# andrewhou1/BlindShadowRemoval

Measured on AMD Instinct MI355X. Metric: images/sec at 256x256 batch inference (GSC generator forward), higher is better.
Workload: dtype f32; 1 GPU; BASELINE configs[1]: batch=32 synthetic 256x256x3 per GPU, full GSC generator fp32 (seeded random-init weights in the ckpt-94 variable layout); global_batch=32, height=256, width=256, parallelism=dp1, forwards_in_flight=1, collective=none

## Files before the change

blindshadowremoval_amd/_lib.py:

```python
from __future__ import annotations

import ctypes
import os
from typing import Optional

from . import build as _build
from .build import LIB_PATH

ABI_VERSION = 8
NUM_CLASSES = 7
CLASS_NAMES = ("conv3x3", "convT3x3", "conv1x1", "attention", "conv7", "glue", "convT3x3_ni2")

_lib: Optional[ctypes.CDLL] = None

c_i, c_v, c_sz, c_s = ctypes.c_int, ctypes.c_void_p, ctypes.c_size_t, ctypes.c_char_p
_BS = [c_i, c_i]
_BLOBS = [c_v, c_sz, c_v, c_sz]

SIGNATURES = {
    "bsr_abi_version": (c_i, None),
    "bsr_last_error": (c_s, None),
    "bsr_source_sha": (c_s, None),
    "bsr_create": (c_i, [ctypes.POINTER(c_v), c_i, c_v, c_sz, c_i]),
    "bsr_destroy": (None, [c_v]),
    "bsr_forward": (c_i, [c_v, c_v, c_v, c_i, c_i, c_i, c_v, c_v, c_v, c_v, c_v]),
    "bsr_forward_packed": (c_i, [c_v, c_v, c_v, c_i, c_i, c_i, c_v, c_v, c_v, c_v]),
    "bsr_forward_tsm": (c_i, [c_v, c_v, c_v, c_v, c_i, c_i, c_i, c_i, c_i, c_v, c_v, c_v, c_v, c_v]),
    "bsr_forward_rgb": (c_i, [c_v, c_v, c_v, c_i, c_i, c_i, c_v, c_v]),
    "bsr_workspace_bytes": (c_sz, [c_i, c_i, c_i]),
    "bsr_handle_workspace_bytes": (c_sz, [c_v, c_i, c_i, c_i]),
    "bsr_reserve": (c_i, [c_v, c_i, c_i, c_i]),
    "bsr_probe": (c_i, [c_v, c_s, c_v, c_sz, ctypes.POINTER(c_i * 4), c_v]),
    "bsr_set_timing": (c_i, [c_v, c_i]),
    "bsr_get_timing": (c_i, [c_v, ctypes.POINTER(ctypes.c_float * NUM_CLASSES), ctypes.POINTER(c_i * NUM_CLASSES)]),
    "bsr_timing_launches": (c_i, [c_v]),
    "bsr_timing_entry": (c_i, [c_v, c_i, c_s, c_sz, ctypes.POINTER(ctypes.c_float), ctypes.POINTER(c_i)]),
    "bsr_clock_trace": (c_i, [c_i, c_v, c_i, c_i, c_v, c_v, c_v]),
    "bsr_check_range": (c_i, [c_v, c_v]),
    "bsr_peek_range": (c_i, [c_v]),
    "bsr_debug_attention": (c_i, [c_v, c_v, c_i, c_i, c_v]),
    "bsr_debug_attention_rgb": (c_i, [c_v, c_v, c_i, c_i, c_v]),
    "bsr_debug_attention_dtype": (c_i, [c_v, c_v, c_i, c_i, c_i, c_v]),
    "bsr_debug_attention_qw": (c_i, [c_v, c_v, c_i, c_i, c_i, c_v]),
    "bsr_debug_attention_split": (c_i, [c_v, c_v, c_i, c_i, c_i, c_v]),
    "bsr_debug_attention_kv1": (c_i, [c_v, c_v, c_i, c_i, c_i, c_v]),
    "bsr_debug_split_qkv": (c_i, [c_v, c_v, c_i, c_i, c_v]),
    "bsr_debug_wino_conv": (c_i, [c_v, c_v, c_v, c_v, c_i, c_i, c_i, c_i, c_v]),
    "bsr_debug_wino_filter": (c_i, [c_v, c_v]),
    "bsr_debug_keys_compose": (c_i, [c_v, c_v, c_v, c_v]),
    "bsr_debug_values_compose": (c_i, [c_v, c_v, c_v, c_v, c_v, c_v]),
    "bsr_prep_rows": (c_i, [c_i, c_v, c_sz, c_sz, c_sz, c_i, c_i, c_v, c_v, c_v]),
    "bsr_prep_groups": (c_i, [c_i, c_v, c_sz, c_sz, c_sz, c_i, c_i, c_i, c_v, c_v, c_v]),
    "bsr_png_unfilter": (c_i, [c_i, c_v, c_sz, c_sz, c_i, c_v]),
    "bsr_png_unfilter_tall": (c_i, [c_i, c_v, c_sz, c_sz, c_i, c_v]),
    "bsr_png_file_bytes": (c_sz, [c_i, c_i]),
    "bsr_png_scratch_bytes": (c_sz, [c_i]),
    "bsr_png_encode": (c_i, [c_i, c_v, c_i, c_i, c_i, c_v, c_sz, c_v, c_v]),
    "bsr_png_encode_figs": (c_i, [c_i, c_i, c_v, c_v, c_v, c_v, c_v, c_v, c_i, c_i, c_i, c_v, c_sz, c_v, c_v]),
    "bsr_crop_faces": (c_i, [c_i, c_v, c_sz, c_sz, c_i, c_i, c_v]),
    "bsr_paste_faces": (c_i, [c_i, c_v, c_sz, c_sz, c_i, c_i, c_v, c_i, c_v, c_i, c_v, c_i, c_i, c_v]),
    "bsr_ucb_post_scratch_bytes": (c_sz, _BS),
    "bsr_ucb_post": (c_i, [c_i, c_v, c_v, c_v, c_i, c_i, c_v, c_v, c_v, c_v, c_v, c_v]),
    "bsr_ucb_post_rgb_scratch_bytes": (c_sz, _BS),
    "bsr_ucb_post_rgb": (c_i, [c_i, c_v, c_v, c_v, c_i, c_i, c_v, c_v, c_v, c_v, c_v, c_v]),
    "bsr_ucb_post_tsm_scratch_bytes": (c_sz, _BS),
    "bsr_ucb_post_tsm": (c_i, [c_i, c_v, c_v, c_v, c_i, c_i, c_v, c_v, c_v, c_v, c_v, c_v, c_v]),
    "bsr_sfw_score_scratch_bytes": (c_sz, _BS),
    "bsr_sfw_score": (c_i, [c_i, c_v, c_i, c_i, c_v, c_v, c_v, c_v, c_v, c_v, c_v]),
    "bsr_shadow_synth_scratch_bytes": (c_sz, _BS),
    "bsr_shadow_synth": (c_i, [c_i, c_v, c_v, c_v, c_v, c_v, c_sz, c_i, c_i, c_v, c_v, c_v, c_v, c_v, c_v, c_v]),
    "bsr_train_losses_scratch_bytes": (c_sz, _BS),
    "bsr_train_losses": (c_i, [c_i, c_v, c_v, c_v, c_v, c_v, c_i, c_i, c_v, c_v, c_v, c_v, c_v, c_v, c_v]),
    "bsr_train_losses_grad_scratch_bytes": (c_sz, _BS),
    "bsr_train_losses_grad_offset": (c_sz, [c_i, c_i, c_i]),
    "bsr_train_losses_grad": (c_i, [c_i, c_v, c_v, c_v, c_v, c_v, c_v, c_i, c_i, c_v, c_v, c_v, c_v, c_v, c_v, c_v, c_v]),
    "bsr_disc_blob_bytes": (c_sz, []),
    "bsr_disc_losses_scratch_bytes": (c_sz, _BS),
    "bsr_disc_act_offset": (c_sz, [c_i, c_i, c_i, c_i]),
    "bsr_disc_losses": (c_i, [c_i, c_v, c_sz, c_v, c_v, c_v, c_i, c_i, c_v, c_v, c_v, c_v, c_v]),
    "bsr_disc_dgrad_blob_bytes": (c_sz, []),
    "bsr_disc_grad_scratch_bytes": (c_sz, _BS),
    "bsr_disc_grad_offset": (c_sz, [c_i, c_i, c_i, c_i]),
    "bsr_disc_gen_grad": (c_i, [c_i] + _BLOBS + [c_v, c_v, c_v, c_v, c_i, c_i, c_v, c_v, c_v, c_v, c_v, c_v]),
    "bsr_debug_disc_gen_grad": (c_i, [c_i] + _BLOBS + [c_v, c_v, c_v, c_v, c_i, c_i, c_v, c_v, c_v, c_v, c_v, c_i, c_v]),
    "bsr_disc_wgrad_blob_bytes": (c_sz, []),
    "bsr_disc_wgrad_scratch_bytes": (c_sz, _BS),
    "bsr_disc_wgrad_floats": (c_sz, []),
    "bsr_disc_wgrad_var_offset": (c_sz, [c_i]),
    "bsr_disc_wgrad_offset": (c_sz, [c_i, c_i, c_i, c_i]),
    "bsr_disc_wgrad": (c_i, [c_i] + _BLOBS + [c_v, c_sz, c_v, c_v, c_v, c_i, c_i, c_v, c_v, c_v, c_v, c_v, c_v]),
    "bsr_debug_disc_wgrad": (c_i, [c_i] + _BLOBS + [c_v, c_sz, c_v, c_v, c_v, c_i, c_i, c_v, c_v, c_v, c_v, c_v, c_i, c_v]),
    "bsr_clr_tail_grad_blob_bytes": (c_sz, []),
    "bsr_clr_tail_grad_scratch_bytes": (c_sz, [c_i, c_i, c_i]),
    "bsr_clr_tail_grad_floats": (c_sz, []),
    "bsr_clr_tail_grad_var_offset": (c_sz, [c_i]),
    "bsr_clr_tail_grad_offset": (c_sz, [c_i, c_i, c_i, c_i]),
    "bsr_clr_tail_grad_partials": (c_i, [c_i, c_i, c_i]),
    "bsr_clr_tail_grad": (c_i, [c_i, c_v, c_sz, c_v, c_v, c_i, c_v, c_v, c_i, c_i, c_i, c_v, c_v, c_v, c_i, c_v, c_v]),
    "bsr_debug_clr_tail_grad": (c_i, [c_i, c_v, c_sz, c_v, c_v, c_i, c_v, c_v, c_i, c_i, c_i, c_v, c_v, c_v, c_i, c_v, c_i, c_v]),
    "bsr_last_f": (c_i, [c_v, ctypes.POINTER(c_v), ctypes.POINTER(c_i), ctypes.POINTER(c_i * 4)]),
# ... 76 lines not shown
```

blindshadowremoval_amd/csrc/bsr_api.hip:

```cpp
#include "../../include/bsr_hip.h"

#include <hip/hip_runtime.h>
#include <stdint.h>
#include <stdio.h>
#include <stdlib.h>
#include <string.h>

#include <initializer_list>
#include <string>
#include <type_traits>
#include <unordered_map>
#include <vector>

#include "attention.h"
#include "attention256.h"
#include "attention_h16.h"
#include "conv3_f16.h"
#include "conv_n16.h"
#include "gemm_nloop.h"
#include "glue_kernels.h"
#include "igemm_conv.h"
#include "igemm_h16.h"
#include "png_kernels.h"
#include "prep_kernels.h"
// ... 124 lines not shown
  p.xa = take(cells * v.cs_a, true);
  p.t1 = take(cells * v.d);
  p.t2 = take(cells * v.d);
  for (int i = 0; i < v.nblk; ++i) p.y3[i] = take(cells * v.cs_y3x);
  p.qkv = take(cells * 3 * v.d);
  for (int i = 0; i < v.nblk; ++i) p.att[i] = take(cells * v.d);
  for (int i = 0; i < v.nblk; ++i) p.r[i] = take(cells * (i < 3 ? v.cs_r : v.cs_h), !v.rgb);
  p.xh = take(cells * v.cs_h, true);
  p.ybuf = take(px * v.cs_y);
  p.qh = take(px * v.cs_qh);
  p.f1 = take(px2 / 16 * 128);
  p.f2 = take(px2 / 4 * 96);
  p.cf = take(px2 * CS_CF);
  p.probe = take(px2 / 64 * 2);
  p.reg32 = take(v.tsm ? cells * 4 : 0);
  p.share = take(v.tsm ? cells * 2 * v.c_r : 0);
  p.yh = take(px1 * 3);
  p.con = take(px1 * 3);
  p.total = off;
  return p;
}

}

struct bsr_handle {
  int device = 0;
  float* d_blob = nullptr;
  float* d_wino = nullptr;
  float* d_keys = nullptr;
  float* d_values = nullptr;
  float* att_scratch = nullptr;
  size_t att_scratch_floats = 0;
  std::unordered_map<std::string, LayerW> layers;
  Variant var = kGSC;
  int dtype = BSR_DTYPE_F32;
  float head_bias[2] = {0.f, 0.f};
  const float* tail_w = nullptr;
  const float* clr_gs_w = nullptr;
  float* ws = nullptr;
  size_t ws_floats = 0;
  Plan plan{};
  const float* rgb_tail_w = nullptr;
  const float* rgb_head_b = nullptr;
  int B = 0, H = 0, W = 0;
  bool ran = false;
  bool att_in_lds = false;
  unsigned* range_flag = nullptr;
  bool fuse_heads = true;
  bool conv1_gemm = true;
  bool att_pv1 = false;
  bool conv3_f16 = true;
  bool fuse_attw = true;
  bool wino_conv2 = true;
  bool keys_conv2 = true;
  bool values_conv2 = true;
  bool att_is_o = false;
  bool timing = false;
  std::vector<hipEvent_t> ev;
  std::vector<int> ev_class;
  std::vector<std::string> ev_name;
  size_t ev_used = 0;
};

namespace {

const char* const kRangeMsg =
    "an activation exceeded the fp16 range (|x| >= 65520) in a forward of this 16-bit-mode handle: its outputs are not trustworthy "
    "(inf / NaN where the fp32 path stays finite).  Re-run those inputs on a BSR_DTYPE_F32 handle; bsr_check_range() clears the condition";

constexpr size_t kWinoFloats = 8 * 16 * 128 * 16;
void wino_filter_transform(const float* direct, float* out) {
  static const double G[4][3] = {{1.0, 0.0, 0.0}, {0.5, 0.5, 0.5}, {0.5, -0.5, 0.5}, {0.0, 0.0, 1.0}};
  for (int k = 0; k < 128; ++k)
    for (int n = 0; n < 128; ++n) {
      double t[4][3];
      for (int x = 0; x < 4; ++x)
        for (int b = 0; b < 3; ++b) {
          double acc = 0.0;
          for (int a = 0; a < 3; ++a) acc += G[x][a] * (double)direct[((size_t)((k / 32) * 9 + a * 3 + b) * 128 + n) * 36 + k % 32];
          t[x][b] = acc;
        }
      for (int x = 0; x < 4; ++x)
        for (int y = 0; y < 4; ++y) {
          double acc = 0.0;
          for (int b = 0; b < 3; ++b) acc += t[x][b] * G[y][b];
          out[((size_t)((k / 16) * 16 + 4 * x + y) * 128 + n) * 16 + k % 16] = (float)acc;
        }
    }
}

constexpr int kKeysN = 288 + 256, kKeysNPad = kKeysN + 64, kC3qNPad = 768;
constexpr size_t kKeysFloats = (size_t)4 * kKeysNPad * 36 + kKeysNPad;
void keys_compose(const float* c3q_w, const float* c3q_b, float* out_w, float* out_b) {
  auto src = [&](int k, int n) -> const float& { return c3q_w[((size_t)(k / 32) * kC3qNPad + n) * 36 + k % 32]; };
  memset(out_w, 0, (size_t)4 * kKeysNPad * 36 * sizeof(float));
  memset(out_b, 0, kKeysNPad * sizeof(float));
  for (int ch = 0; ch < 4; ++ch) {
    memcpy(out_w + (size_t)ch * kKeysNPad * 36, c3q_w + (size_t)ch * kC3qNPad * 36, (size_t)288 * 36 * sizeof(float));
    memcpy(out_w + ((size_t)ch * kKeysNPad + 416) * 36, c3q_w + ((size_t)ch * kC3qNPad + 544) * 36, (size_t)128 * 36 * sizeof(float));
  }
  memcpy(out_b, c3q_b, 288 * sizeof(float));
  memcpy(out_b + 416, c3q_b + 544, 128 * sizeof(float));
  for (int m = 0; m < 128; ++m) {
    for (int k = 0; k < 128; ++k) {
      double acc = 0.0;
      for (int c = 0; c < 128; ++c) acc += (double)src(k, 288 + c) * (double)src(m, 416 + c);
// ... 196 lines not shown
      const int most = (tiles + NI - 1) / NI;
      kNSplit = want < 2 ? 2 : (want > most ? most : want);
#ifdef BSR_NL_NSPLIT
      kNSplit = BSR_NL_NSPLIT > most ? most : BSR_NL_NSPLIT;
#endif
    }
    if (image == nullptr) rc = find_layer(h, name, NCH, 1, 36, (tiles + NI - 1) * 32, &l);
    else if (image->nchunk == NCH && image->ldp == 36 && image->n_pad >= (tiles + NI - 1) * 32) l = *image;
    else rc = fail(BSR_ERR_ARG, std::string("layer '") + name + "': the handle's image does not fit the kernel");
    if (rc != BSR_OK) return;
    if (pixels % C::BM != 0) { rc = fail(BSR_ERR_ARG, std::string("layer '") + name + "': pixel count is not a multiple of 128"); return; }
    bsr::ConvArgs a = gemm_args(l, in, in_cs, out, out_cs, n_store, act);
    a.res1 = res1; a.res1_cs = res1_cs; a.res1_c = res1_c;
    a.out2 = out2; a.out2_cs = out2_cs; a.n_split = n_split; a.n_store1 = n_store1; a.out2_gap_at = out2_gap_at; a.out2_gap = out2_gap;
    a.out2_split = (h->dtype != BSR_DTYPE_F32 && out2 != nullptr) ? 1 : 0;
    begin(cls, name);
    if (h->dtype == BSR_DTYPE_F32)
      check(bsr::launch_gemm_nloop<NI, NCH, 0, MINW>(a, pixels, kNSplit, s), name);
    else if constexpr (MINW == 2)
      check(bsr::launch_gemm_nloop<NI, NCH, 2>(a, pixels, kNSplit, s), name);
    else
      rc = fail(BSR_ERR_ARG, std::string("layer '") + name + "': the RGB bottleneck GEMMs are fp32 only");
    end();
  }
  template <int NCH>
  void gemm_all_n(const char* name, const float* in, size_t pixels, float* out) {
    if (rc != BSR_OK) return;
    LayerW l;
    rc = find_layer(h, name, NCH, 1, 36, 128, &l);
    if (rc != BSR_OK) return;
    begin(K_CONV1, name);
    check(bsr::launch_gemm_nloop<4, NCH, 2, 1>(gemm_args(l, in, NCH * 32, out, 128, 128, 1), pixels, 1, s), name);
    end();
  }

  void stem(const float* in, int H, int W, float* out) {
    if (rc != BSR_OK) return;
    LayerW l;
    rc = find_layer(h, "conv1", 1, 7, h->dtype != BSR_DTYPE_F32 ? 36 : 28, 32, &l);
    if (rc != BSR_OK) return;
    bsr::StemArgs a{in, out, l.w, l.b, H, W, 0, 0, 0, h->range_flag};
    begin(K_CONV7, "conv1");
    with_dtype(h->dtype, [&](auto prec, auto half) { check(bsr::launch_stem7<4, prec.value, half.value>(a, h->B, s), "conv1"); });
    end();
  }

  void wino(const char* name, int i, const float* in, int H, int W, float* out, int out_cs = 128) {
    if (rc != BSR_OK) return;
    LayerW l;
    rc = find_layer(h, name, 4, 9, 36, 128, &l);
    if (rc != BSR_OK) return;
    if (H % 4 != 0 || W % 32 != 0) { rc = fail(BSR_ERR_ARG, std::string("layer '") + name + "': feature map is not a multiple of the 4x32 tile"); return; }
    begin(K_CONV3, name);
    check(bsr::launch_wino_conv2(wino_args(in, out, h->d_wino + (size_t)i * kWinoFloats, l.b, H, W, out_cs), h->B, s), name);
    end();
  }

  void conv71(const char* name, const float* in, int in_cs, int k_pad, int H, int W, float* out, int out_cs) {
    if (rc != BSR_OK) return;
    LayerW l;
    rc = find_layer(h, name, k_pad / 32, 7, 36, 32, &l);
    if (rc != BSR_OK) return;
    if (H % 4 != 0 || W % 32 != 0) { rc = fail(BSR_ERR_ARG, std::string("layer '") + name + "': image is not a multiple of the 4x32 tile"); return; }
    bsr::ConvArgs a{};
    a.in = in; a.in_cs = in_cs; a.in_coff = 0; a.H = H; a.W = W;
    a.out = out; a.out_cs = out_cs; a.out_coff = 0; a.Ho = H; a.Wo = W;
    a.w = l.w; a.bias = l.b; a.nchunk = l.nchunk; a.n_pad = l.n_pad; a.n_store = 32;
    a.pad_t = 3; a.pad_l = 0; a.act = 0;
    begin(K_CONV7, name);
    check(bsr::launch_igemm_conv<7, 1, 1, false, 4, 32, 4, 1, 1, 1, 32, 1>(a, h->B, s), name);
    end();
  }

  void heads(const float* y, int H, int W, float* qh, const float* inputs, float* gs, float* mask22, size_t npix) {
    if (rc != BSR_OK) return;
    LayerW l;
    rc = find_layer(h, "heads", 2, 7, 36, 16, &l);
    if (rc != BSR_OK) return;
    if (l.n_pad != 16) { rc = fail(BSR_ERR_BLOB, "layer 'heads' must be packed with n_pad 16"); return; }
    if (H % 8 != 0 || W % 32 != 0) { rc = fail(BSR_ERR_ARG, "layer 'heads': image is not a multiple of its tile"); return; }
    bsr::ConvN16Args a{};
    a.in = y; a.in_cs = 64; a.H = H; a.W = W; a.w = l.w; a.bias = l.b; a.out = qh; a.out_cs = 16; a.act = 0;
    a.pad_t = 3; a.pad_l = 0;
    a.inputs = inputs; a.gs_out = gs; a.mask22 = mask22; a.b_mask = h->head_bias[0]; a.b_con = h->head_bias[1];
    a.range_flag = h->range_flag;
    int resident = 0;
    check(bsr::launch_conv_n16<7, 1, false, false, 2, 0, false, true>(a, h->B, s, &resident), "heads");
    const bool fuse = rc == BSR_OK && h->fuse_heads && bsr::conv_n16_fuse_pays(h->B, H, 8, resident);
    begin(K_CONV7, "heads");
    with_dtype(h->dtype, [&](auto prec, auto half) {
      if (fuse) check(bsr::launch_conv_n16<7, 1, false, false, 2, prec.value, half.value, true>(a, h->B, s), "heads");
      else check(bsr::launch_conv_n16<7, 1, false, false, 2, prec.value, half.value>(a, h->B, s), "heads");
    });
    end();
    if (fuse) return;
    begin(K_GLUE, "heads_post");
    hipLaunchKernelGGL(bsr::heads_post_kernel, dim3((unsigned)((npix + 255) / 256)), dim3(256), 0, s, qh, inputs, h->head_bias[0], h->head_bias[1], gs,
                       mask22, W, npix);
    check(hipGetLastError(), "heads_post");
    end();
  }

  template <int KH, int KW, bool GS, bool TAIL, int RW>
  void conv16(int cls, const char* name, const float* in, int in_cs, int H, int W, float* out, int out_cs, int act, const float* gs,
              const float* inputs, float* con_rgb, float* dif, float* packed = nullptr) {
    if (rc != BSR_OK) return;
    LayerW l;
// ... 43 lines not shown
}

template <typename T>
int read_records(const unsigned char* blob, size_t off, int n, hipStream_t s, std::vector<T>* out) {
  out->resize((size_t)n);
  HIP_TRY(hipMemcpyAsync(out->data(), blob + off, (size_t)n * sizeof(T), hipMemcpyDeviceToHost, s));
  HIP_TRY(hipStreamSynchronize(s));
  return BSR_OK;
}

}

extern "C" {

int bsr_abi_version(void) { return 8; }

#ifndef BSR_SRC_SHA
#define BSR_SRC_SHA "unhashed"
#endif
static const char kSrcShaTag[] = "BSR_SRC_SHA=" BSR_SRC_SHA;
const char* bsr_source_sha(void) { return kSrcShaTag + 12; }

const char* bsr_last_error(void) { return g_last_error.c_str(); }

size_t bsr_workspace_bytes(int B, int H, int W) {
  if (B <= 0 || H <= 0 || W <= 0) return 0;
  return make_plan(B, H, W, kGSC).total * sizeof(float);
}

int bsr_create(bsr_handle** out, int device, const void* packed_weights, size_t nbytes, int dtype) {
  if (out == nullptr || packed_weights == nullptr) return fail(BSR_ERR_ARG, "bsr_create: null argument");
  *out = nullptr;
  if (dtype != BSR_DTYPE_F32 && dtype != BSR_DTYPE_F16 && dtype != BSR_DTYPE_F32X3)
    return fail(BSR_ERR_ARG, "bsr_create: dtype must be BSR_DTYPE_F32, BSR_DTYPE_F16 or BSR_DTYPE_F32X3");
  if (nbytes < sizeof(BlobHeader)) return fail(BSR_ERR_BLOB, "bsr_create: blob shorter than its header");
  const uint8_t* blob = static_cast<const uint8_t*>(packed_weights);
  BlobHeader hd;
  memcpy(&hd, blob, sizeof hd);
  if (hd.magic != kBlobMagic || hd.version != kBlobVersion) return fail(BSR_ERR_BLOB, "bsr_create: bad blob magic/version");
  if ((int)hd.reserved != dtype) return fail(BSR_ERR_BLOB, "bsr_create: the blob was packed for another dtype (pack_generator(weights, dtype) must match bsr_create's dtype)");
  const size_t table_end = sizeof(BlobHeader) + (size_t)hd.n_entries * sizeof(BlobEntry);
  if (table_end > nbytes) return fail(BSR_ERR_BLOB, "bsr_create: blob entry table exceeds blob size");
  DeviceGuard guard(device);
  HIP_TRY(guard.err);
  bsr_handle* h = new bsr_handle();
  h->device = device;
  h->dtype = dtype;
  h->att_pv1 = dtype == BSR_DTYPE_F16;
  const struct { const char* env; bool* on; } switches[] = {{"BSR_FUSE_HEADS", &h->fuse_heads}, {"BSR_FUSE_ATTW", &h->fuse_attw}, {"BSR_CONV3_F16", &h->conv3_f16},
                                                            {"BSR_CONV1_GEMM", &h->conv1_gemm}, {"BSR_WINO_CONV2", &h->wino_conv2},
                                                            {"BSR_KEYS_CONV2", &h->keys_conv2}, {"BSR_VALUES_CONV2", &h->values_conv2}};
  for (const auto& sw : switches)
    if (const char* e_ = getenv(sw.env)) *sw.on = atoi(e_) != 0;
  hipError_t e = hipMalloc(reinterpret_cast<void**>(&h->d_blob), nbytes);
  if (e == hipSuccess) e = hipMemcpy(h->d_blob, blob, nbytes, hipMemcpyHostToDevice);
  if (e != hipSuccess) {
    if (h->d_blob) hipFree(h->d_blob);
    delete h;
    return fail(BSR_ERR_HIP, std::string("bsr_create: weight upload: ") + hipGetErrorString(e));
  }
  for (uint32_t i = 0; i < hd.n_entries; ++i) {
    BlobEntry en;
    memcpy(&en, blob + sizeof(BlobHeader) + (size_t)i * sizeof(BlobEntry), sizeof en);
    en.name[sizeof(en.name) - 1] = 0;
    if (en.offset % 16 != 0 || en.offset + en.nfloats * 4 > nbytes) {
      bsr_destroy(h);
      return fail(BSR_ERR_BLOB, std::string("bsr_create: entry '") + en.name + "' is out of bounds or misaligned");
    }
    std::string nm(en.name);
    const float* dptr = reinterpret_cast<const float*>(reinterpret_cast<const uint8_t*>(h->d_blob) + en.offset);
    if (nm == "heads.bias") {
      if (en.nfloats != 2) { bsr_destroy(h); return fail(BSR_ERR_BLOB, "bsr_create: heads.bias must hold 2 floats"); }
      memcpy(h->head_bias, blob + en.offset, 8);
    } else if (nm == "clr_conv1.gs") {
      if (en.nfloats != 256) { bsr_destroy(h); return fail(BSR_ERR_BLOB, "bsr_create: clr_conv1.gs must hold 16x16 floats"); }
      h->clr_gs_w = dptr;
    } else if (nm == "rgb.tail") {
      if (en.nfloats != 7 * 7 * 3 * 3 + 3) { bsr_destroy(h); return fail(BSR_ERR_BLOB, "bsr_create: rgb.tail must hold 7x7x3x3 + 3 floats"); }
      h->rgb_tail_w = dptr;
    } else if (nm == "rgb.head_bias") {
      if (en.nfloats != 3) { bsr_destroy(h); return fail(BSR_ERR_BLOB, "bsr_create: rgb.head_bias must hold 3 floats"); }
      h->rgb_head_b = dptr;
    } else if (nm == "tail.w") {
      if (en.nfloats != 16 * 16 + 16 + 48 + 3) { bsr_destroy(h); return fail(BSR_ERR_BLOB, "bsr_create: tail.w has the wrong size"); }
      h->tail_w = dptr;
    } else if (nm.size() > 2 && nm.compare(nm.size() - 2, 2, ".w") == 0) {
      LayerW& l = h->layers[nm.substr(0, nm.size() - 2)];
      l.w = dptr;
      l.nchunk = en.dims[0]; l.taps = en.dims[1]; l.n_pad = en.dims[2]; l.ldp = en.dims[3];
      if ((uint64_t)l.nchunk * l.taps * l.n_pad * l.ldp != en.nfloats) {
        bsr_destroy(h);
        return fail(BSR_ERR_BLOB, std::string("bsr_create: entry '") + en.name + "' dims do not match its size");
      }
    } else if (nm.size() > 2 && nm.compare(nm.size() - 2, 2, ".b") == 0) {
      h->layers[nm.substr(0, nm.size() - 2)].b = dptr;
    }
  }
  if (h->layers.count("rgb_head") != 0) {
    if (dtype != BSR_DTYPE_F32) {
      bsr_destroy(h);
      return fail(BSR_ERR_ARG, "bsr_create: these are RGB-baseline weights (model_RGB.py), which run in BSR_DTYPE_F32 only: BSR_DTYPE_F32X3 and BSR_DTYPE_F16 are not provided for them");
    }
    if (h->rgb_tail_w == nullptr || h->rgb_head_b == nullptr) { bsr_destroy(h); return fail(BSR_ERR_BLOB, "bsr_create: RGB blob lacks 'rgb.tail' / 'rgb.head_bias'"); }
    h->var = kRGB;
    *out = h;
    return BSR_OK;
// ... 1015 lines not shown
  return BSR_OK;
}

int bsr_debug_attention_split(const void* qkv_split, float* y, int B, int tokens, int pv1, void* stream) {
  if (qkv_split == nullptr || y == nullptr) return fail(BSR_ERR_ARG, "bsr_debug_attention_split: null argument");
  if (B <= 0 || tokens <= 0 || tokens % 128 != 0) return fail(BSR_ERR_ARG, "bsr_debug_attention_split: tokens must be a positive multiple of 128");
  HIP_TRY(bsr::launch_nonlocal_attention_h16(static_cast<const float*>(qkv_split), y, B, tokens, static_cast<hipStream_t>(stream), pv1 != 0));
  return BSR_OK;
}

int bsr_debug_attention_dtype(const float* qkv, float* y, int B, int tokens, int dtype, void* stream) {
  if (qkv == nullptr || y == nullptr) return fail(BSR_ERR_ARG, "bsr_debug_attention: null argument");
  if (B <= 0 || tokens <= 0 || tokens % 128 != 0) return fail(BSR_ERR_ARG, "bsr_debug_attention: tokens must be a positive multiple of 128");
  if (dtype == BSR_DTYPE_F32) {
    HIP_TRY(bsr::launch_nonlocal_attention(qkv, y, B, tokens, static_cast<hipStream_t>(stream)));
  } else if (dtype == BSR_DTYPE_F32X3 || dtype == BSR_DTYPE_F16) {
    void* tmp = nullptr;
    HIP_TRY(hipMalloc(&tmp, (size_t)B * tokens * bsr::kA4TokBytes));
    int rc = bsr_debug_split_qkv(qkv, tmp, B, tokens, stream);
    if (rc == BSR_OK) rc = bsr_debug_attention_split(tmp, y, B, tokens, 0, stream);
    hipError_t e = hipStreamSynchronize(static_cast<hipStream_t>(stream));
    hipFree(tmp);
    if (rc != BSR_OK) return rc;
    HIP_TRY(e);
  } else {
    return fail(BSR_ERR_ARG, "bsr_debug_attention: unknown dtype");
  }
  return BSR_OK;
}

int bsr_debug_attention_qw(const float* qkv, float* y, int B, int tokens, int qw, void* stream) {
  if (qkv == nullptr || y == nullptr) return fail(BSR_ERR_ARG, "bsr_debug_attention_qw: null argument");
  if (B <= 0 || tokens <= 0 || tokens % 128 != 0) return fail(BSR_ERR_ARG, "bsr_debug_attention_qw: tokens must be a positive multiple of 128");
  if (qw != 0 && qw != 1 && qw != 2 && qw != 4) return fail(BSR_ERR_ARG, "bsr_debug_attention_qw: qw must be 0 (automatic), 1, 2 or 4 query waves per workgroup");
  HIP_TRY(bsr::launch_nonlocal_attention(qkv, y, B, tokens, static_cast<hipStream_t>(stream), qw));
  return BSR_OK;
}

int bsr_debug_attention_kv1(const float* qkv2, float* y, int B, int tokens, int qw, void* stream) {
  if (qkv2 == nullptr || y == nullptr) return fail(BSR_ERR_ARG, "bsr_debug_attention_kv1: null argument");
  if (B <= 0 || tokens <= 0 || tokens % 128 != 0) return fail(BSR_ERR_ARG, "bsr_debug_attention_kv1: tokens must be a positive multiple of 128");
  if (qw != 0 && qw != 1 && qw != 2 && qw != 4) return fail(BSR_ERR_ARG, "bsr_debug_attention_kv1: qw must be 0 (automatic), 1, 2 or 4 query waves per workgroup");
  HIP_TRY(bsr::launch_nonlocal_attention<true>(qkv2, y, B, tokens, static_cast<hipStream_t>(stream), qw));
  return BSR_OK;
}

int bsr_debug_attention_rgb(const float* qkv, float* y, int B, int tokens, void* stream) {
  if (qkv == nullptr || y == nullptr) return fail(BSR_ERR_ARG, "bsr_debug_attention_rgb: null argument");
  if (B <= 0 || tokens <= 0 || tokens % 32 != 0) return fail(BSR_ERR_ARG, "bsr_debug_attention_rgb: tokens must be a positive multiple of 32");
  HIP_TRY(bsr::launch_nonlocal_attention256(qkv, y, B, tokens, static_cast<hipStream_t>(stream)));
  return BSR_OK;
}

int bsr_debug_wino_conv(const float* x, const float* w, const float* bias, float* y, int B, int H, int W, int nw, void* stream) {
  if (x == nullptr || w == nullptr || bias == nullptr || y == nullptr) return fail(BSR_ERR_ARG, "bsr_debug_wino_conv: null argument");
  if (B <= 0 || H <= 0 || W <= 0 || H % 4 != 0 || W % 32 != 0) return fail(BSR_ERR_ARG, "bsr_debug_wino_conv: H must be a positive multiple of 4 and W of 32");
  if ((long long)B * H * W * 128 * 4 >= (1LL << 31)) return fail(BSR_ERR_ARG, "bsr_debug_wino_conv: tensor too large");
  if (nw != 0 && nw != 2 && nw != 4) return fail(BSR_ERR_ARG, "bsr_debug_wino_conv: nw must be 0 (automatic), 2 or 4 waves per workgroup");
  HIP_TRY(bsr::launch_wino_conv2(wino_args(x, y, w, bias, H, W), B, static_cast<hipStream_t>(stream), nw));
  return BSR_OK;
}

int bsr_debug_wino_filter(const float* direct, float* out) {
  if (direct == nullptr || out == nullptr) return fail(BSR_ERR_ARG, "bsr_debug_wino_filter: null argument");
  wino_filter_transform(direct, out);
  return BSR_OK;
}

int bsr_debug_keys_compose(const float* c3q_w, const float* c3q_b, float* out_w, float* out_b) {
  if (c3q_w == nullptr || c3q_b == nullptr || out_w == nullptr || out_b == nullptr) return fail(BSR_ERR_ARG, "bsr_debug_keys_compose: null argument");
  keys_compose(c3q_w, c3q_b, out_w, out_b);
  return BSR_OK;
}

int bsr_debug_values_compose(const float* c3q_w, const float* c3q_b, const float* w_w, const float* w_b, float* out_w, float* out_b) {
  if (c3q_w == nullptr || c3q_b == nullptr || w_w == nullptr || w_b == nullptr || out_w == nullptr || out_b == nullptr)
    return fail(BSR_ERR_ARG, "bsr_debug_values_compose: null argument");
  values_compose(c3q_w, c3q_b, w_w, w_b, out_w, out_b);
  return BSR_OK;
}

int bsr_debug_attention(const float* qkv, float* y, int B, int tokens, void* stream) {
  return bsr_debug_attention_dtype(qkv, y, B, tokens, BSR_DTYPE_F32, stream);
}

struct ProbeSrc { size_t off; int hh, ww, cs, coff, c; bool half; int derive; };

static int probe_index(const std::string& nm, const char* prefix, int n) {
  const size_t len = strlen(prefix);
  if (nm.size() == len + 1 && nm.compare(0, len, prefix) == 0 && nm[len] >= '0' && nm[len] < '0' + n) return nm[len] - '0';
  return -1;
}

static int probe_src_rgb(const bsr_handle* h, const std::string& nm, ProbeSrc* src) {
  const Plan& p = h->plan;
  const int H = h->H, W = h->W;
  int i;
  if (nm == "x1") *src = {p.x1, H, W, 32, 0, 32};
  else if (nm == "x2") *src = {p.c3, H / 2, W / 2, RGB_CS_C3, 128, 64};
  else if (nm == "x3") *src = {p.c2, H / 4, W / 4, RGB_CS_C2, 192, 64};
  else if (nm == "x0") *src = {p.xa, H / 8, W / 8, RGB_CS_A, 0, 99};
  else if ((i = probe_index(nm, "res", 3)) >= 0) *src = {p.r[i], H / 8, W / 8, RGB_CS_R, 0, 513};
  else if ((i = probe_index(nm, "att", 3)) >= 0) *src = {p.att[i], H / 8, W / 8, RGB_D, 0, RGB_D};
  else if ((i = probe_index(nm, "y3x", 3)) >= 0) *src = {p.y3[i], H / 8, W / 8, RGB_CS_R, 0, 513};
  else if (nm == "up1") *src = {p.c2, H / 4, W / 4, RGB_CS_C2, 0, 192};
  else if (nm == "up2") *src = {p.c3, H / 2, W / 2, RGB_CS_C3, 0, 128};
  else if (nm == "up3") *src = {p.ybuf, H, W, 128, 0, 128};
  else if (nm == "y") *src = {p.yh, H, W, 3, 0, 3};
  else if (nm == "con") *src = {p.con, H, W, 3, 0, 3};
  else return fail(BSR_ERR_STATE, "bsr_probe: unknown probe '" + nm + "' for an RGB handle");
  return BSR_OK;
}

// ... 106 lines not shown
```

blindshadowremoval_amd/csrc/wino_conv2.h:

```cpp
#pragma once
#include <hip/hip_runtime.h>
#include <stdint.h>

#include "mfma_common.h"

namespace bsr {

struct WinoArgs {
  const float* in;
  float* out;
  const float* w;
  const float* bias;
  int H, W;
  int in_cs, out_cs;
  int tiles_x, tiles_y;
  int act;
};

template <int NW>
struct WinoCfg {
  static constexpr int NT = NW * 64;
  static constexpr int CC = 16;
  static constexpr int LDP = CC + 4;
  static constexpr int K = 128, N = 128, NCHUNK = K / CC;
  static constexpr int SPC = 8;
  static constexpr int NSTEPS = NCHUNK * SPC;
  static constexpr int BN = NW * 32;
  static constexpr int V_POS = 32 * LDP;
  static constexpr int V_FLOATS = 16 * V_POS;
  static constexpr int U_POS = BN * LDP;
  static constexpr int U_FLOATS = 2 * U_POS;
  static constexpr int SMEM_BYTES = (2 * V_FLOATS + 3 * U_FLOATS) * 4;
  static constexpr int IT = 256 / NT;
  static_assert(NW == 4 || NW == 2, "4 waves (128 channels) or 2 waves (64 channels) per workgroup");
  static_assert(SMEM_BYTES <= 160 * 1024, "LDS budget");
};

template <int NW>
__global__ __launch_bounds__(NW * 64, 1) void wino_conv2_kernel(WinoArgs p) {
  using C = WinoCfg<NW>;
  constexpr int NT = C::NT, LDP = C::LDP, IT = C::IT, SPC = C::SPC, NSTEPS = C::NSTEPS;
  typedef unsigned u32x4_t __attribute__((ext_vector_type(4)));
  typedef unsigned u32x2_t __attribute__((ext_vector_type(2)));
  extern __shared__ __attribute__((aligned(16))) float smem[];
  float* s_v = smem;
  float* s_u = smem + 2 * C::V_FLOATS;

  const int tid = threadIdx.x;
  const int lane = tid & 63;
  const int wave = __builtin_amdgcn_readfirstlane(tid >> 6);
  const int h = lane >> 5, r = lane & 31;

  int bid = blockIdx.x;
  const int tile_x = bid % p.tiles_x;
  bid /= p.tiles_x;
  const int tile_y = bid % p.tiles_y;
  const int img = bid / p.tiles_y;
  const int n0 = blockIdx.y * C::BN;
  const int y0 = tile_y * 4, x0 = tile_x * 32;
  const float* in_img = p.in + (size_t)img * p.H * p.W * p.in_cs;
  const __amdgpu_buffer_rsrc_t in_rsrc = make_rsrc(in_img);

  unsigned in_goff[IT][16];
  int v_loff[IT];
#pragma unroll
  for (int it = 0; it < IT; ++it) {
    const int item = tid + it * NT;
    const int patch = item >> 3, cp = item & 7;
    const int py = patch >> 4, px = patch & 15;
#pragma unroll
    for (int a = 0; a < 4; ++a)
#pragma unroll
      for (int b = 0; b < 4; ++b) {
        const int iy = y0 + 2 * py - 1 + a, ix = x0 + 2 * px - 1 + b;
        const bool ok = iy >= 0 && iy < p.H && ix >= 0 && ix < p.W;
        in_goff[it][4 * a + b] = ok ? (unsigned)(((iy * p.W + ix) * p.in_cs + 2 * cp) * 4) : kLaneOff;
      }
    v_loff[it] = patch * LDP + 2 * cp;
  }
  unsigned w_goff[2];
  int w_loff[2];
#pragma unroll
  for (int j = 0; j < 2; ++j) {
    const int e = tid + j * NT;
    w_goff[j] = (unsigned)(e * 16);
    w_loff[j] = (e >> 2) * LDP + (e & 3) * 4;
  }
  const __amdgpu_buffer_rsrc_t w_rsrc = make_rsrc(p.w + (size_t)n0 * C::CC);
  constexpr unsigned kPosBytes = (unsigned)(C::N * C::CC * 4);
  const float bias_n = p.bias[n0 + wave * 32 + r];

  auto fetch_in = [&](int chunk, f32x2 (&d)[IT][16]) {
// ... 13 lines not shown
      d[it][8 + b] = d2 - d1;
      d[it][12 + b] = d1 - d3;
    }
  };
  auto in_cols_store = [&](int v_off, const f32x2 (&d)[IT][16], int a) {
#pragma unroll
    for (int it = 0; it < IT; ++it) {
      const f32x2 w0 = d[it][4 * a], w1 = d[it][4 * a + 1], w2 = d[it][4 * a + 2], w3 = d[it][4 * a + 3];
      float* dst = s_v + v_off + v_loff[it] + 4 * a * C::V_POS;
      *reinterpret_cast<f32x2*>(dst) = w0 - w2;
      *reinterpret_cast<f32x2*>(dst + C::V_POS) = w1 + w2;
      *reinterpret_cast<f32x2*>(dst + 2 * C::V_POS) = w2 - w1;
      *reinterpret_cast<f32x2*>(dst + 3 * C::V_POS) = w1 - w3;
    }
  };
  auto fetch_w = [&](int t, f32x4 (&regs)[4]) {
#pragma unroll
    for (int pl = 0; pl < 2; ++pl)
#pragma unroll
      for (int j = 0; j < 2; ++j)
        regs[2 * pl + j] = __builtin_bit_cast(f32x4, (u32x4_t)__builtin_amdgcn_raw_buffer_load_b128(w_rsrc, w_goff[j], (unsigned)(2 * t + pl) * kPosBytes, 0));
  };
  auto store_w1 = [&](int u_off, const f32x4 (&regs)[4], int i) {
    *reinterpret_cast<f32x4*>(s_u + u_off + (i >> 1) * C::U_POS + w_loff[i & 1]) = regs[i];
  };

  f32x2 d[IT][16];
  f32x4 w_regs[2][4];
  int u_cur = 0, u_n1 = C::U_FLOATS, u_n2 = 2 * C::U_FLOATS;
  int v_cur = 0, v_nxt = C::V_FLOATS;
  fetch_in(0, d);
  fetch_w(0, w_regs[0]);
  fetch_w(1, w_regs[1]);
#pragma unroll
  for (int b = 0; b < 4; ++b) in_rows(d, b);
#pragma unroll
  for (int a = 0; a < 4; ++a) in_cols_store(0, d, a);
#pragma unroll
  for (int i = 0; i < 4; ++i) store_w1(u_cur, w_regs[0], i);
#pragma unroll
  for (int i = 0; i < 4; ++i) store_w1(u_n1, w_regs[1], i);
  fetch_w(2, w_regs[1]);
  __syncthreads();

  f32x16 acc[16];
#pragma unroll
  for (int q = 0; q < 16; ++q)
#pragma unroll
    for (int i = 0; i < 16; ++i) acc[q][i] = 0.f;
  acc[5] = bias_tile(h, bias_n);

  const int a_base = r * LDP + 4 * h;
  const int b_base = (wave * 32 + r) * LDP + 4 * h;
  f32x4 af[2], bf[2];
  auto read_frags = [&](int slot, int v_off, int u_off) {
    af[slot] = *reinterpret_cast<const f32x4*>(s_v + a_base + v_off);
    bf[slot] = *reinterpret_cast<const f32x4*>(s_u + b_base + u_off);
  };
  read_frags(0, v_cur, u_cur);

  for (int ch = 0; ch < C::NCHUNK; ++ch) {
    const int ch1 = ch + 1 < C::NCHUNK ? ch + 1 : C::NCHUNK - 1;
#pragma unroll
    for (int s = 0; s < SPC; ++s) {
      const int t = ch * SPC + s;
      fetch_w(t + 3 < NSTEPS ? t + 3 : NSTEPS - 1, w_regs[s & 1]);
      if (s == 0) fetch_in(ch1, d);
      __builtin_amdgcn_sched_barrier(0);
#pragma unroll
      for (int q = 0; q < 4; ++q) {
        const int cur = q & 1, nxt = cur ^ 1;
        const int pl = q >> 1;
        if (q < 3) {
          const int pl1 = (q + 1) >> 1, g1 = (q + 1) & 1;
          read_frags(nxt, v_cur + (2 * s + pl1) * C::V_POS + g1 * 8, u_cur + pl1 * C::U_POS + g1 * 8);
        } else if (s + 1 < SPC) {
          read_frags(nxt, v_cur + (2 * s + 2) * C::V_POS, u_n1);
        } else {
          read_frags(nxt, v_nxt, u_n1);
        }
        store_w1(u_n2, w_regs[(s + 1) & 1], q);
        if (s == SPC - 3) in_rows(d, q);
        if (s == SPC - 2) in_cols_store(v_nxt, d, q);
        __builtin_amdgcn_sched_barrier(0);
#pragma unroll
        for (int j = 0; j < 4; ++j)
          acc[2 * s + pl] = __builtin_amdgcn_mfma_f32_32x32x2f32(af[cur][j], bf[cur][j], acc[2 * s + pl], 0, 0, 0);
        __builtin_amdgcn_sched_barrier(0);
      }
      __syncthreads();
      { const int tu = u_cur; u_cur = u_n1; u_n1 = u_n2; u_n2 = tu; }
      if (s == SPC - 1) { const int tv = v_cur; v_cur = v_nxt; v_nxt = tv; }
    }
  }

  const float alpha = p.act ? kLeakyAlpha : 1.f;
  const unsigned cs4 = (unsigned)p.out_cs * 4u;
  const __amdgpu_buffer_rsrc_t orsrc =
      make_rsrc(p.out + ((size_t)img * p.H * p.W + (size_t)y0 * p.W + x0) * p.out_cs + n0 + wave * 32);
  const unsigned lane_out = (unsigned)(8 * h) * cs4 + (unsigned)r * 4u;
#pragma unroll
  for (int v = 0; v < 16; ++v) {
    float t0[4], t1[4];
#pragma unroll
    for (int nu = 0; nu < 4; ++nu) {
      t0[nu] = (acc[nu][v] + acc[4 + nu][v]) + acc[8 + nu][v];
      t1[nu] = (acc[4 + nu][v] - acc[8 + nu][v]) - acc[12 + nu][v];
    }
    f32x2 y0v = f32x2{(t0[0] + t0[1]) + t0[2], (t0[1] - t0[2]) - t0[3]};
    f32x2 y1v = f32x2{(t1[0] + t1[1]) + t1[2], (t1[1] - t1[2]) - t1[3]};
    const f32x2 s0 = y0v * alpha, s1 = y1v * alpha;
    const int prow = 2 * (v >> 3), pcol = 2 * (8 * ((v >> 2) & 1) + (v & 3));
#pragma unroll
    for (int i = 0; i < 2; ++i)
#pragma unroll
      for (int j = 0; j < 2; ++j) {
        const float x = i ? y1v[j] : y0v[j], ax = i ? s1[j] : s0[j];
        const unsigned soff = (unsigned)((prow + i) * p.W + pcol + j) * cs4;
        __builtin_amdgcn_raw_buffer_store_b32(__float_as_uint(__builtin_amdgcn_fmed3f(x, ax, 3.4028234664e38f)), orsrc, lane_out, soff, 0);
      }
  }
}

inline int wino_conv2_auto_nw(int batch, int H, int W) {
  const long long tiles = (long long)batch * (H / 4) * (W / 32);
  return 2 * tiles <= device_cu_count() ? 2 : 4;
}

template <int NW>
inline hipError_t launch_wino_conv2_nw(WinoArgs a, int batch, hipStream_t stream) {
  using C = WinoCfg<NW>;
  auto kern = wino_conv2_kernel<NW>;
  static PerDeviceOnce once;
  const int dev = PerDeviceOnce::current();
  if (dev < 0 || !once.done[dev]) {
    hipError_t e = hipFuncSetAttribute(reinterpret_cast<const void*>(kern), hipFuncAttributeMaxDynamicSharedMemorySize, C::SMEM_BYTES);
    if (e != hipSuccess) return e;
    if (dev >= 0) once.done[dev] = true;
  }
  a.tiles_x = a.W / 32;
  a.tiles_y = a.H / 4;
  dim3 grid(a.tiles_x * a.tiles_y * batch, 4 / NW);
  hipLaunchKernelGGL(kern, grid, dim3(C::NT), C::SMEM_BYTES, stream, a);
  return hipGetLastError();
}

inline hipError_t launch_wino_conv2(const WinoArgs& a, int batch, hipStream_t stream, int nw = 0) {
  if (nw == 0) nw = wino_conv2_auto_nw(batch, a.H, a.W);
  return nw == 2 ? launch_wino_conv2_nw<2>(a, batch, stream) : launch_wino_conv2_nw<4>(a, batch, stream);
}

}
```

include/bsr_hip.h:

```cpp
#ifndef BSR_HIP_H_
#define BSR_HIP_H_

#include <stddef.h>

#ifdef __cplusplus
extern "C" {
#endif

typedef struct bsr_handle bsr_handle;

#define BSR_OK 0
#define BSR_ERR_ARG 1
#define BSR_ERR_BLOB 2
#define BSR_ERR_HIP 3
#define BSR_ERR_STATE 4
#define BSR_ERR_RANGE 5

#define BSR_DTYPE_F32 0
#define BSR_DTYPE_F16 1
#define BSR_DTYPE_F32X3 2

int bsr_create(bsr_handle** out, int device, const void* packed_weights, size_t nbytes, int dtype);

int bsr_forward(bsr_handle* h, const float* inputs, const float* uv, int B, int H, int W,
// ... 103 lines not shown
                         const float* f, int f_cs, const float* d_f, int B, int H, int W, float* d_x, float* grads, int keep, void* scratch, void* stream);
int bsr_debug_clr_decoder_grad(int device, const void* d_blob, size_t blob_bytes, const float* x, int x_cs, const float* f1, int f1_cs, const float* f2,
                               int f2_cs, const float* f, int f_cs, const float* d_f, int B, int H, int W, float* d_x, float* grads, int keep, void* scratch,
                               int stop_after, void* stream);

size_t bsr_vgg_blob_bytes(void);
size_t bsr_vgg_scratch_bytes(int B, int S);
size_t bsr_vgg_act_offset(int B, int S, int layer);
int bsr_vgg_per_loss(int device, const void* d_blob, size_t blob_bytes, const float* gt, const float* con_rgb, int B, int S, double* sums,
                     float* loss1, void* scratch, void* stream);

size_t bsr_vgg_dgrad_blob_bytes(void);
size_t bsr_vgg_grad_scratch_bytes(int B, int S);
size_t bsr_vgg_grad_offset(int B, int S, int which);
int bsr_vgg_per_loss_grad(int device, const void* d_blob, size_t blob_bytes, const void* d_dgrad_blob, size_t dgrad_bytes, const float* gt,
                          const float* con_rgb, const float* upstream, int B, int S, double* sums, float* loss1, float* grad, void* scratch,
                          void* stream);
int bsr_debug_vgg_per_loss_grad(int device, const void* d_blob, size_t blob_bytes, const void* d_dgrad_blob, size_t dgrad_bytes,
                                const float* gt, const float* con_rgb, const float* upstream, int B, int S, double* sums, float* loss1,
                                float* grad, void* scratch, int stop_after, void* stream);

size_t bsr_png_file_bytes(int H, int W);
size_t bsr_png_scratch_bytes(int B);
int bsr_png_encode(int device, const unsigned char* pixels, int B, int H, int W, unsigned char* out, size_t out_stride, void* scratch,
                   void* stream);

int bsr_png_encode_figs(int device, int n_figs, const float* const* figs, const float* const* muls, const float* scales, const int* channels,
                        const int* pixel_strides, const int* mul_strides, int B, int H, int Wf, unsigned char* out, size_t out_stride, void* scratch,
                        void* stream);

size_t bsr_ucb_post_scratch_bytes(int B, int S);
int bsr_ucb_post(int device, const float* rows10, const unsigned char* masks, const float* boxes, int B, int S, float* losses,
                 unsigned char* strips, float* figs, int* status, void* scratch, void* stream);

size_t bsr_ucb_post_rgb_scratch_bytes(int B, int S);
int bsr_ucb_post_rgb(int device, const float* rows9, const unsigned char* masks, const float* boxes, int B, int S, float* losses,
                     unsigned char* strips, float* figs, int* status, void* scratch, void* stream);

size_t bsr_sfw_score_scratch_bytes(int B, int S);
int bsr_sfw_score(int device, const float* rows3, int B, int S, float* losses, double* auc, float* pred, float* label, int* status,
                  void* scratch, void* stream);

size_t bsr_ucb_post_tsm_scratch_bytes(int B, int S);
int bsr_ucb_post_tsm(int device, const float* rows, const unsigned char* masks, const float* boxes, int B, int S, float* losses,
                     double* nose_stats, unsigned char* strips, float* figs, int* status, void* scratch, void* stream);

int bsr_debug_attention(const float* qkv, float* y, int B, int tokens, void* stream);
int bsr_debug_attention_rgb(const float* qkv, float* y, int B, int tokens, void* stream);
int bsr_debug_attention_dtype(const float* qkv, float* y, int B, int tokens, int dtype, void* stream);
int bsr_debug_split_qkv(const float* qkv, void* qkv_split, int B, int tokens, void* stream);
int bsr_debug_attention_split(const void* qkv_split, float* y, int B, int tokens, int pv1, void* stream);
int bsr_debug_attention_qw(const float* qkv, float* y, int B, int tokens, int qw, void* stream);
int bsr_debug_wino_conv(const float* x, const float* w, const float* bias, float* y, int B, int H, int W, int nw, void* stream);
int bsr_debug_wino_filter(const float* direct, float* out);
int bsr_debug_keys_compose(const float* c3q_w, const float* c3q_b, float* out_w, float* out_b);
int bsr_debug_values_compose(const float* c3q_w, const float* c3q_b, const float* w_w, const float* w_b, float* out_w, float* out_b);
int bsr_debug_attention_kv1(const float* qkv2, float* y, int B, int tokens, int qw, void* stream);

int bsr_clock_trace(int device, unsigned long long* out, int samples, int spin, const int* stop, int* taken, void* stream);

void bsr_destroy(bsr_handle* h);

const char* bsr_last_error(void);

int bsr_abi_version(void);

const char* bsr_source_sha(void);

#ifdef __cplusplus
}
#endif
#endif
```

Measured before the change: 7002 images/sec.

## Add two-chain MFMA accumulator variant and sched_group_barrier interleaving to Winograd conv

Adds a CHAINS template parameter to the Winograd conv kernel. With two chains, two accumulator sets get independent MFMA chains so back-to-back MFMA dependencies are hidden. Both paths now use sched_group_barrier to interleave MFMA with LDS reads and writes, global loads and VALU work, where before hard sched_barriers separated these phases. Two chains stay opt-in via BSR_WINO_CHAINS, but the default one-chain path also gets the new interleaved schedule, which changes codegen for the default run.

```diff
diff --git a/blindshadowremoval_amd/_lib.py b/blindshadowremoval_amd/_lib.py
--- a/blindshadowremoval_amd/_lib.py
+++ b/blindshadowremoval_amd/_lib.py
@@ -46,6 +46,7 @@
     "bsr_debug_attention_kv1": (c_i, [c_v, c_v, c_i, c_i, c_i, c_v]),
     "bsr_debug_split_qkv": (c_i, [c_v, c_v, c_i, c_i, c_v]),
     "bsr_debug_wino_conv": (c_i, [c_v, c_v, c_v, c_v, c_i, c_i, c_i, c_i, c_v]),
+    "bsr_debug_wino_conv_chains": (c_i, [c_v, c_v, c_v, c_v, c_i, c_i, c_i, c_i, c_i, c_v]),
     "bsr_debug_wino_filter": (c_i, [c_v, c_v]),
     "bsr_debug_keys_compose": (c_i, [c_v, c_v, c_v, c_v]),
     "bsr_debug_values_compose": (c_i, [c_v, c_v, c_v, c_v, c_v, c_v]),
diff --git a/blindshadowremoval_amd/csrc/bsr_api.hip b/blindshadowremoval_amd/csrc/bsr_api.hip
--- a/blindshadowremoval_amd/csrc/bsr_api.hip
+++ b/blindshadowremoval_amd/csrc/bsr_api.hip
@@ -200,6 +200,7 @@
   bool conv3_f16 = true;
   bool fuse_attw = true;
   bool wino_conv2 = true;
+  int wino_chains = 1;
   bool keys_conv2 = true;
   bool values_conv2 = true;
   bool att_is_o = false;
@@ -502,7 +503,7 @@
     if (rc != BSR_OK) return;
     if (H % 4 != 0 || W % 32 != 0) { rc = fail(BSR_ERR_ARG, std::string("layer '") + name + "': feature map is not a multiple of the 4x32 tile"); return; }
     begin(K_CONV3, name);
-    check(bsr::launch_wino_conv2(wino_args(in, out, h->d_wino + (size_t)i * kWinoFloats, l.b, H, W, out_cs), h->B, s), name);
+    check(bsr::launch_wino_conv2(wino_args(in, out, h->d_wino + (size_t)i * kWinoFloats, l.b, H, W, out_cs), h->B, s, 0, h->wino_chains), name);
     end();
   }
 
@@ -652,6 +653,7 @@
                                                             {"BSR_KEYS_CONV2", &h->keys_conv2}, {"BSR_VALUES_CONV2", &h->values_conv2}};
   for (const auto& sw : switches)
     if (const char* e_ = getenv(sw.env)) *sw.on = atoi(e_) != 0;
+  if (const char* e_ = getenv("BSR_WINO_CHAINS")) h->wino_chains = atoi(e_) == 2 ? 2 : 1;
   hipError_t e = hipMalloc(reinterpret_cast<void**>(&h->d_blob), nbytes);
   if (e == hipSuccess) e = hipMemcpy(h->d_blob, blob, nbytes, hipMemcpyHostToDevice);
   if (e != hipSuccess) {
@@ -1773,13 +1775,18 @@
   return BSR_OK;
 }
 
-int bsr_debug_wino_conv(const float* x, const float* w, const float* bias, float* y, int B, int H, int W, int nw, void* stream) {
+int bsr_debug_wino_conv_chains(const float* x, const float* w, const float* bias, float* y, int B, int H, int W, int nw, int chains, void* stream) {
   if (x == nullptr || w == nullptr || bias == nullptr || y == nullptr) return fail(BSR_ERR_ARG, "bsr_debug_wino_conv: null argument");
   if (B <= 0 || H <= 0 || W <= 0 || H % 4 != 0 || W % 32 != 0) return fail(BSR_ERR_ARG, "bsr_debug_wino_conv: H must be a positive multiple of 4 and W of 32");
   if ((long long)B * H * W * 128 * 4 >= (1LL << 31)) return fail(BSR_ERR_ARG, "bsr_debug_wino_conv: tensor too large");
   if (nw != 0 && nw != 2 && nw != 4) return fail(BSR_ERR_ARG, "bsr_debug_wino_conv: nw must be 0 (automatic), 2 or 4 waves per workgroup");
-  HIP_TRY(bsr::launch_wino_conv2(wino_args(x, y, w, bias, H, W), B, static_cast<hipStream_t>(stream), nw));
-  return BSR_OK;
+  if (chains != 1 && chains != 2) return fail(BSR_ERR_ARG, "bsr_debug_wino_conv_chains: chains must be 1 or 2 accumulator chains");
+  HIP_TRY(bsr::launch_wino_conv2(wino_args(x, y, w, bias, H, W), B, static_cast<hipStream_t>(stream), nw, chains));
+  return BSR_OK;
+}
+
+int bsr_debug_wino_conv(const float* x, const float* w, const float* bias, float* y, int B, int H, int W, int nw, void* stream) {
+  return bsr_debug_wino_conv_chains(x, w, bias, y, B, H, W, nw, 1, stream);
 }
 
 int bsr_debug_wino_filter(const float* direct, float* out) {
diff --git a/blindshadowremoval_amd/csrc/wino_conv2.h b/blindshadowremoval_amd/csrc/wino_conv2.h
--- a/blindshadowremoval_amd/csrc/wino_conv2.h
+++ b/blindshadowremoval_amd/csrc/wino_conv2.h
@@ -36,8 +36,11 @@
   static_assert(SMEM_BYTES <= 160 * 1024, "LDS budget");
 };
 
-template <int NW>
+constexpr int kSchedValu = 0x002, kSchedMfma = 0x008, kSchedVmemRead = 0x020, kSchedDsRead = 0x100, kSchedDsWrite = 0x200;
+
+template <int NW, int CHAINS = 1>
 __global__ __launch_bounds__(NW * 64, 1) void wino_conv2_kernel(WinoArgs p) {
+  static_assert(CHAINS == 1 || CHAINS == 2, "one or two accumulator chains in the matrix loop");
   using C = WinoCfg<NW>;
   constexpr int NT = C::NT, LDP = C::LDP, IT = C::IT, SPC = C::SPC, NSTEPS = C::NSTEPS;
   typedef unsigned u32x4_t __attribute__((ext_vector_type(4)));
@@ -157,12 +160,13 @@
 
   const int a_base = r * LDP + 4 * h;
   const int b_base = (wave * 32 + r) * LDP + 4 * h;
-  f32x4 af[2], bf[2];
-  auto read_frags = [&](int slot, int v_off, int u_off) {
-    af[slot] = *reinterpret_cast<const f32x4*>(s_v + a_base + v_off);
-    bf[slot] = *reinterpret_cast<const f32x4*>(s_u + b_base + u_off);
-  };
-  read_frags(0, v_cur, u_cur);
+  f32x4 af[2][CHAINS], bf[2][CHAINS];
+  auto read_frags = [&](int slot, int pl, int v_off, int u_off) {
+    af[slot][pl] = *reinterpret_cast<const f32x4*>(s_v + a_base + v_off);
+    bf[slot][pl] = *reinterpret_cast<const f32x4*>(s_u + b_base + u_off);
+  };
+#pragma unroll
+  for (int pl = 0; pl < CHAINS; ++pl) read_frags(0, pl, v_cur + pl * C::V_POS, u_cur + pl * C::U_POS);
 
   for (int ch = 0; ch < C::NCHUNK; ++ch) {
     const int ch1 = ch + 1 < C::NCHUNK ? ch + 1 : C::NCHUNK - 1;
@@ -171,27 +175,68 @@
       const int t = ch * SPC + s;
       fetch_w(t + 3 < NSTEPS ? t + 3 : NSTEPS - 1, w_regs[s & 1]);
       if (s == 0) fetch_in(ch1, d);
-      __builtin_amdgcn_sched_barrier(0);
-#pragma unroll
-      for (int q = 0; q < 4; ++q) {
-        const int cur = q & 1, nxt = cur ^ 1;
-        const int pl = q >> 1;
-        if (q < 3) {
-          const int pl1 = (q + 1) >> 1, g1 = (q + 1) & 1;
-          read_frags(nxt, v_cur + (2 * s + pl1) * C::V_POS + g1 * 8, u_cur + pl1 * C::U_POS + g1 * 8);
-        } else if (s + 1 < SPC) {
-          read_frags(nxt, v_cur + (2 * s + 2) * C::V_POS, u_n1);
-        } else {
-          read_frags(nxt, v_nxt, u_n1);
+      if constexpr (CHAINS == 2) {
+#pragma unroll
+        for (int g = 0; g < 2; ++g) {
+          const int cur = g, nxt = g ^ 1;
+#pragma unroll
+          for (int pl = 0; pl < 2; ++pl) {
+            if (g == 0) read_frags(nxt, pl, v_cur + (2 * s + pl) * C::V_POS + 8, u_cur + pl * C::U_POS + 8);
+            else if (s + 1 < SPC) read_frags(nxt, pl, v_cur + (2 * s + 2 + pl) * C::V_POS, u_n1 + pl * C::U_POS);
+            else read_frags(nxt, pl, v_nxt + pl * C::V_POS, u_n1 + pl * C::U_POS);
+          }
+#pragma unroll
+          for (int q = 2 * g; q < 2 * g + 2; ++q) {
+            store_w1(u_n2, w_regs[(s + 1) & 1], q);
+            if (s == SPC - 3) in_rows(d, q);
+            if (s == SPC - 2) in_cols_store(v_nxt, d, q);
+          }
+#pragma unroll
+          for (int j = 0; j < 4; ++j)
+#pragma unroll
+            for (int pl = 0; pl < 2; ++pl)
+              acc[2 * s + pl] = __builtin_amdgcn_mfma_f32_32x32x2f32(af[cur][pl][j], bf[cur][pl][j], acc[2 * s + pl], 0, 0, 0);
+#pragma unroll
+          for (int i = 0; i < 8; ++i) {
+            __builtin_amdgcn_sched_group_barrier(kSchedMfma, 1, 0);
+            if (g == 0 && s == 0) __builtin_amdgcn_sched_group_barrier(kSchedVmemRead, (4 + 16 * IT + 7) / 8, 0);
+            if (g == 0 && s != 0 && i < 4) __builtin_amdgcn_sched_group_barrier(kSchedVmemRead, 1, 0);
+            if (i < 4) __builtin_amdgcn_sched_group_barrier(kSchedDsRead, 1, 0);
+            __builtin_amdgcn_sched_group_barrier(kSchedDsWrite, IT + 1, 0);
+            __builtin_amdgcn_sched_group_barrier(kSchedValu, IT + 2, 0);
+          }
+          __builtin_amdgcn_sched_barrier(0);
         }
-        store_w1(u_n2, w_regs[(s + 1) & 1], q);
-        if (s == SPC - 3) in_rows(d, q);
-        if (s == SPC - 2) in_cols_store(v_nxt, d, q);
-        __builtin_amdgcn_sched_barrier(0);
-#pragma unroll
-        for (int j = 0; j < 4; ++j)
-          acc[2 * s + pl] = __builtin_amdgcn_mfma_f32_32x32x2f32(af[cur][j], bf[cur][j], acc[2 * s + pl], 0, 0, 0);
-        __builtin_amdgcn_sched_barrier(0);
+      } else {
+#pragma unroll
+        for (int q = 0; q < 4; ++q) {
+          const int cur = q & 1, nxt = cur ^ 1;
+          const int pl = q >> 1;
+          if (q < 3) {
+            const int pl1 = (q + 1) >> 1, g1 = (q + 1) & 1;
+            read_frags(nxt, 0, v_cur + (2 * s + pl1) * C::V_POS + g1 * 8, u_cur + pl1 * C::U_POS + g1 * 8);
+          } else if (s + 1 < SPC) {
+            read_frags(nxt, 0, v_cur + (2 * s + 2) * C::V_POS, u_n1);
+          } else {
+            read_frags(nxt, 0, v_nxt, u_n1);
+          }
+          store_w1(u_n2, w_regs[(s + 1) & 1], q);
+          if (s == SPC - 3) in_rows(d, q);
+          if (s == SPC - 2) in_cols_store(v_nxt, d, q);
+#pragma unroll
+          for (int j = 0; j < 4; ++j)
+            acc[2 * s + pl] = __builtin_amdgcn_mfma_f32_32x32x2f32(af[cur][0][j], bf[cur][0][j], acc[2 * s + pl], 0, 0, 0);
+#pragma unroll
+          for (int i = 0; i < 4; ++i) {
+            __builtin_amdgcn_sched_group_barrier(kSchedMfma, 1, 0);
+            if (q == 0 && s == 0) __builtin_amdgcn_sched_group_barrier(kSchedVmemRead, (4 + 16 * IT) / 4, 0);
+            if (q == 0 && s != 0) __builtin_amdgcn_sched_group_barrier(kSchedVmemRead, 1, 0);
+            if (i < 2) __builtin_amdgcn_sched_group_barrier(kSchedDsRead, 1, 0);
+            __builtin_amdgcn_sched_group_barrier(kSchedDsWrite, IT + 1, 0);
+            __builtin_amdgcn_sched_group_barrier(kSchedValu, IT + 2, 0);
+          }
+          __builtin_amdgcn_sched_barrier(0);
+        }
       }
       __syncthreads();
       { const int tu = u_cur; u_cur = u_n1; u_n1 = u_n2; u_n2 = tu; }
@@ -232,10 +277,10 @@
   return 2 * tiles <= device_cu_count() ? 2 : 4;
 }
 
-template <int NW>
+template <int NW, int CHAINS>
 inline hipError_t launch_wino_conv2_nw(WinoArgs a, int batch, hipStream_t stream) {
   using C = WinoCfg<NW>;
-  auto kern = wino_conv2_kernel<NW>;
+  auto kern = wino_conv2_kernel<NW, CHAINS>;
   static PerDeviceOnce once;
   const int dev = PerDeviceOnce::current();
   if (dev < 0 || !once.done[dev]) {
@@ -250,9 +295,10 @@
   return hipGetLastError();
 }
 
-inline hipError_t launch_wino_conv2(const WinoArgs& a, int batch, hipStream_t stream, int nw = 0) {
+inline hipError_t launch_wino_conv2(const WinoArgs& a, int batch, hipStream_t stream, int nw = 0, int chains = 1) {
   if (nw == 0) nw = wino_conv2_auto_nw(batch, a.H, a.W);
-  return nw == 2 ? launch_wino_conv2_nw<2>(a, batch, stream) : launch_wino_conv2_nw<4>(a, batch, stream);
-}
-
-}
+  if (chains == 2) return nw == 2 ? launch_wino_conv2_nw<2, 2>(a, batch, stream) : launch_wino_conv2_nw<4, 2>(a, batch, stream);
+  return nw == 2 ? launch_wino_conv2_nw<2, 1>(a, batch, stream) : launch_wino_conv2_nw<4, 1>(a, batch, stream);
+}
+
+}
diff --git a/include/bsr_hip.h b/include/bsr_hip.h
--- a/include/bsr_hip.h
+++ b/include/bsr_hip.h
@@ -179,6 +179,7 @@
 int bsr_debug_attention_split(const void* qkv_split, float* y, int B, int tokens, int pv1, void* stream);
 int bsr_debug_attention_qw(const float* qkv, float* y, int B, int tokens, int qw, void* stream);
 int bsr_debug_wino_conv(const float* x, const float* w, const float* bias, float* y, int B, int H, int W, int nw, void* stream);
+int bsr_debug_wino_conv_chains(const float* x, const float* w, const float* bias, float* y, int B, int H, int W, int nw, int chains, void* stream);
 int bsr_debug_wino_filter(const float* direct, float* out);
 int bsr_debug_keys_compose(const float* c3q_w, const float* c3q_b, float* out_w, float* out_b);
 int bsr_debug_values_compose(const float* c3q_w, const float* c3q_b, const float* w_w, const float* w_b, float* out_w, float* out_b);
```

After: 7058 images/sec, median of 6. No clear change (+0.8%).
